# LucasAlegre/morl-baselines

Measured on NVIDIA B200. Metric: envelope_q_updates_per_sec, higher is better.
Workload: dtype f32

## Files before the change

### include/morl_b200.h

```cpp
#ifndef MORL_B200_H_
#define MORL_B200_H_

#include <stddef.h>
#include <stdint.h>

#ifdef __cplusplus
extern "C" {
#endif

#define MORL_B200_VERSION 100

#if defined(__GNUC__)
#define MORL_API __attribute__((visibility("default")))
#else
#define MORL_API
#endif

#define MORL_OK 0
#define MORL_ERR_NULL (-1)
#define MORL_ERR_SHAPE (-2)
#define MORL_ERR_ALIGN (-3)
#define MORL_ERR_UNSUPPORTED (-4)
#define MORL_ERR_NO_DEVICE (-5)

// ... 66 lines not shown
                                 void* stream);
MORL_API int morl_front_unpack_f64(const double* gathered, int world, int d, int cap, int n_extra, double* pts_out, double* meta_out, void* stream);

MORL_API int morl_hypervolume_f64(const double* pts, const uint8_t* keep, int n, int d, const double* ref, double* out, void* stream);

MORL_API int morl_polyak_f32(const float* const* params, float* const* targets, const int64_t* sizes, int n_tensors,
                    int64_t max_size, double tau, void* stream);


MORL_API int morl_sumtree_walk_f64(const double* tree, int n_levels, const double* u, int n, int scale_by_root, long long* out_index, void* stream);
MORL_API int morl_sumtree_batch_set_f64(double* tree, int n_levels, const long long* index, const double* priority, int n, int* err_flag,
                                        void* stream);
MORL_API int morl_sumtree_set_f64(double* tree, int n_levels, long long index, double priority, int use_min_priority, const double* min_priority,
                                  int* err_flag, void* stream);
MORL_API int morl_per_priority_f32(const float* raw, int n, float alpha, double* min_priority, double* prio64, float* prio32, void* stream);

#define MORL_FMT_BF16X3 0
#define MORL_FMT_F16X2 1
#define MORL_SPLIT_MAX_JOBS 16
typedef struct MorlSplitJob {
    const float* src;
    void* dst_planes;
    long long plane_stride;
    float* scale;
    int rows, cols, ld_src, transpose, rows_pad, ldp;
    int auto_scale, target_exp;
} MorlSplitJob;
MORL_API int morl_plane_overflow_count(int reset);
MORL_API int morl_amax_scale_f32(const float* src, long long n, int target_exp, float* scale_out, void* workspace, void* stream);
MORL_API int morl_split_planes_multi(int fmt, const MorlSplitJob* jobs, int n_jobs, void* stream);
// ... 72 lines not shown
```

### morl_baselines_b200/_lib.py

```python

from __future__ import annotations

import ctypes as C
import os

HERE = os.path.dirname(os.path.abspath(__file__))
LIB_PATH = os.path.join(HERE, "csrc", "libmorl_b200.so")

DOT_UNFUSED, DOT_FMA, DOT_PAIRFMA = 0, 1, 2
MAP_TILE, MAP_BLOCK = 0, 1
ROWS_REFERENCE, ROWS_BMAJOR = 0, 1
AC_ELEMENTWISE_MIN, AC_SCALAR_MIN, AC_ARGMIN_GATHER = 0, 1, 2
MAX_D = 8
FMT_BF16X3, FMT_F16X2 = 0, 1

_vp, _i, _f, _d, _i64, _sz = C.c_void_p, C.c_int, C.c_float, C.c_double, C.c_int64, C.c_size_t

SIGNATURES = {
    "morl_version": (_i, []),
    "morl_last_error": (C.c_char_p, []),
    "morl_device_sm_count": (_i, []),
    "morl_envelope_td_f32": (_i, [_vp, _vp, _vp, _vp, _vp, _f, _i, _i, _i, _i, _i, _i, _vp, _vp, _vp, _vp]),
    "morl_greedy_td_f32": (_i, [_vp, _vp, _vp, _i, _i, _vp, _vp, _i, _i, _f, _i, _i, _i, _i, _vp, _vp, _vp]),
    "morl_critic_min_td_f32": (_i, [_vp, _i, _vp, _i, _i, _vp, _vp, _i, _i, _f, _i, _i, _i, _i, _vp, _vp, _vp]),
    "morl_gpi_envelope_f32": (_i, [_vp, _i, _vp, _i, _i, _vp, _vp, _i, _i, _f, _i, _i, _i, _i, _i, _vp, _vp, _vp, _vp]),
    "morl_actor_critic_td_f32": (_i, [_vp, _i, _vp, _i, _i, _vp, _vp, _vp, _f, _f, _i, _i, _i, _vp, _vp]),
    "morl_td_workspace_bytes": (_sz, [_i]),
    "morl_td_mse_priority_f32": (_i, [_vp, _vp, _vp, _vp, _f, _vp, _i, _i, _i, _i, _i, _vp, _vp, _vp, _vp, _vp, _vp]),
    "morl_td_huber_priority_f32": (_i, [_vp, _i, _vp, _i, _vp, _vp, _vp, _i, _i, _f, _i, _i, _i, _i, _vp, _vp, _vp, _vp, _vp]),
    "morl_host_sumtree_walk": (_i, [_vp, _i, _vp, _i, _vp]),
    "morl_host_sumtree_batch_set": (_i, [_vp, _i, _vp, _vp, _i]),
    "morl_host_gather_rows": (_i, [_vp, C.c_longlong, _vp, _i, _vp]),
    "morl_host_gather_u8_to_i32": (_i, [_vp, C.c_longlong, _vp, _i, _vp]),
    "morl_sumtree_walk_f64": (_i, [_vp, _i, _vp, _i, _i, _vp, _vp]),
    "morl_sumtree_batch_set_f64": (_i, [_vp, _i, _vp, _vp, _i, _vp, _vp]),
    "morl_sumtree_set_f64": (_i, [_vp, _i, C.c_longlong, _d, _i, _vp, _vp, _vp]),
    "morl_per_priority_f32": (_i, [_vp, _i, _f, _vp, _vp, _vp, _vp]),
    "morl_replay_gather": (_i, [_vp, _vp, _vp, _vp, _vp, _vp, _i, _i, _i, _i, _i, _i64, _vp, _vp, _vp, _vp, _vp, _vp]),
    "morl_pareto_mask_f32": (_i, [_vp, _i, _i, _i, _vp, _vp]),
    "morl_pareto_mask_f64": (_i, [_vp, _i, _i, _i, _vp, _vp]),
    "morl_front_pack_f64": (_i, [_vp, _vp, _i, _i, _i, _vp, _i, _vp, _vp]),
    "morl_front_unpack_f64": (_i, [_vp, _i, _i, _i, _i, _vp, _vp, _vp]),
    "morl_hypervolume_f64": (_i, [_vp, _vp, _i, _i, _vp, _vp, _vp]),
    "morl_polyak_f32": (_i, [_vp, _vp, _vp, _i, _i64, _d, _vp]),
    "morl_plane_overflow_count": (_i, [_i]),
    "morl_amax_scale_f32": (_i, [_vp, C.c_longlong, _i, _vp, _vp, _vp]),
    "morl_split_planes_multi": (_i, [_i, _vp, _i, _vp]),
    "morl_split_planes": (_i, [_i, _vp, _i, _i, _i, _i, _vp, _i, _i, C.c_longlong, _vp, _vp]),
    "morl_gemm_planes_f32": (_i, [_i, _vp, C.c_longlong, _vp, _vp, C.c_longlong, _vp, _i, _i, _i, _i, _vp, _i, _vp, _i, _vp, _i, _vp, _i, C.c_longlong,
                                  _vp, _i, _i, _vp, _vp, _vp]),
    "morl_gemm_chain_supported": (_i, [_i, _i, _i]),
    "morl_gemm_chain_f32": (_i, [_i, _i, _i, _vp, C.c_longlong, _vp, _vp, C.c_longlong, _vp, _vp, _i, _vp, _vp, _i, _i, _i, _vp]),
# ... 69 lines not shown
```

### morl_baselines_b200/common/prioritized_buffer.py

```python

from __future__ import annotations

import numpy as np
import torch as th

from .. import _lib
from .buffer import ReplayBuffer, ReplayBufferSamplesNp


class SumTree:

    def __init__(self, max_size):
        self.n_levels = int(np.ceil(np.log2(max_size))) + 1
        self._alloc(np.zeros((1 << self.n_levels) - 1))

    def _alloc(self, flat):
        self._flat = np.ascontiguousarray(flat, dtype=np.float64)
        self.nodes = [self._flat[(1 << l) - 1 : (1 << (l + 1)) - 1] for l in range(self.n_levels)]
        self._lib = _lib.load()

    def __getstate__(self):
        return {"n_levels": self.n_levels, "flat": self._flat}

    def __setstate__(self, state):
# ... 154 lines not shown
            obs, act, rew, nobs, done = self.gather_device(idxes)
            return obs, act, rew, nobs, done, th.from_numpy(idxes)
        tup = ReplayBufferSamplesNp(self.obs[idxes], self.actions[idxes], self.rewards[idxes], self.next_obs[idxes], self.dones[idxes], idxes)
        if to_tensor:
            return tuple(map(lambda x: th.tensor(x).to(device), tup))
        return tup

    def sample_obs(self, batch_size, to_tensor=False, device=None):
        idxes = self.tree.sample(batch_size)
        return th.tensor(self.obs[idxes]).to(device) if to_tensor else self.obs[idxes]

    def update_priorities(self, idxes, priorities):
        self.min_priority = max(self.min_priority, priorities.max())
        self.tree.batch_set(np.asarray(idxes), priorities)

    def update_priorities_dev(self, idx_dev, raw_dev, alpha: float, prio64_dev, prio32_dev=None):
        if not self.tree_on_device:
            raise _lib.MorlB200Error("update_priorities_dev needs tree_on_device=True")
        lib = _lib.load()
        st = th.cuda.current_stream().cuda_stream
        _lib.check(lib.morl_per_priority_f32(raw_dev.data_ptr(), raw_dev.shape[0], float(alpha), self._min_p_dev.data_ptr(), prio64_dev.data_ptr(),
                                             None if prio32_dev is None else prio32_dev.data_ptr(), st), "morl_per_priority_f32")
        self.tree.batch_set_dev(idx_dev, prio64_dev)

    def get_all_data(self, max_samples=None, to_tensor=False, device=None):
        if max_samples is not None and max_samples < self.size:
            inds = np.random.choice(self.size, max_samples, replace=False)
        else:
            inds = np.arange(self.size)
        tup = (self.obs[inds], self.actions[inds], self.rewards[inds], self.next_obs[inds], self.dones[inds])
        if to_tensor:
            return tuple(map(lambda x: th.tensor(x).to(device), tup))
        return tup
```

### morl_baselines_b200/csrc/api.cu

```cuda
#include <stdlib.h>
#include <stdarg.h>
#include <string.h>

#include "common.cuh"

namespace morl {

static thread_local char g_err[512] = "";

void set_error(const char* fmt, ...) {
    va_list ap;
    va_start(ap, fmt);
    vsnprintf(g_err, sizeof(g_err), fmt, ap);
    va_end(ap);
}

int check_launch(const char* what) {
    cudaError_t e = cudaPeekAtLastError();
    if (e != cudaSuccess) {
        (void)cudaGetLastError();
        set_error("%s: %s", what, cudaGetErrorString(e));
        return static_cast<int>(e);
    }
    return MORL_OK;
}

bool pdl_enabled() {
    static const bool on = [] { const char* e = getenv("MORL_PDL"); return e && e[0] == '1'; }();
    return on;
}

}

extern "C" {

int morl_version(void) { return MORL_B200_VERSION; }

const char* morl_last_error(void) { return morl::g_err; }

int morl_device_sm_count(void) {
    int dev = 0;
    cudaError_t e = cudaGetDevice(&dev);
    if (e != cudaSuccess) {
        (void)cudaGetLastError();
        morl::set_error("morl_device_sm_count: no CUDA device (%s)", cudaGetErrorString(e));
        return MORL_ERR_NO_DEVICE;
// ... 13 lines not shown
```

### morl_baselines_b200/csrc/common.cuh

```cuda
#pragma once
#include <cuda_runtime.h>
#include <math.h>
#include <stdint.h>
#include <stdio.h>
#include <string.h>

#include "../../include/morl_b200.h"

namespace morl {

void set_error(const char* fmt, ...);
int check_launch(const char* what);

#define MORL_REQUIRE(cond, code, ...)    \
    do {                                 \
        if (!(cond)) {                   \
            ::morl::set_error(__VA_ARGS__); \
            return (code);               \
        }                                \
    } while (0)

static inline bool aligned16(const void* p) { return (reinterpret_cast<uintptr_t>(p) & 15u) == 0; }

__device__ __forceinline__ void pdl_enter() {
    asm volatile("griddepcontrol.launch_dependents;" ::: "memory");
    asm volatile("griddepcontrol.wait;" ::: "memory");
}

bool pdl_enabled();

template <typename... KArgs, typename... Args>
static inline void launch_k(void (*kernel)(KArgs...), dim3 grid, dim3 block, size_t smem, cudaStream_t stream, Args&&... args) {
    cudaLaunchConfig_t cfg;
    memset(&cfg, 0, sizeof(cfg));
    cfg.gridDim = grid;
    cfg.blockDim = block;
    cfg.dynamicSmemBytes = smem;
    cfg.stream = stream;
    cudaLaunchAttribute attr[1];
    attr[0].id = cudaLaunchAttributeProgrammaticStreamSerialization;
    attr[0].val.programmaticStreamSerializationAllowed = 1;
    cfg.attrs = attr;
    cfg.numAttrs = pdl_enabled() ? 1 : 0;
    cudaLaunchKernelEx(&cfg, kernel, static_cast<KArgs>(args)...);
// ... 79 lines not shown
```

### morl_baselines_b200/csrc/gemm_planes.cu

```cuda
#include <cuda.h>
#include <cuda_bf16.h>
#include <cuda_fp16.h>
#include <stdlib.h>
#include <string.h>

#include "common.cuh"
#include "gemm_tc.cuh"

namespace morl {

constexpr int kGemmBM = 128;
constexpr int kGemmThreads = 320;

__device__ unsigned int g_plane_overflow;


__device__ __forceinline__ void note_overflow(float amax) {
    if (amax > 65504.f) atomicAdd(&g_plane_overflow, 1u);
}

#define MORL_DISPATCH_FMT(F_, ...)                                                         \
    switch (F_) {                                                                          \
        case MORL_FMT_BF16X3: { constexpr int kFmt = MORL_FMT_BF16X3; __VA_ARGS__; } break; \
        case MORL_FMT_F16X2: { constexpr int kFmt = MORL_FMT_F16X2; __VA_ARGS__; } break;   \
// ... 1249 lines not shown
#pragma unroll
    for (int j = 0; j < 8; ++j) red[threadIdx.y][threadIdx.x][j] = acc[j];
    __syncthreads();
    if (threadIdx.y == 0 && h0 < H) {
#pragma unroll
        for (int j = 0; j < 8; ++j) {
            float t = 0.f;
#pragma unroll
            for (int y = 0; y < 8; ++y) t += red[y][threadIdx.x][j];
            dU[(size_t)b * H + h0 + j] = t * inv;
        }
    }
}

constexpr int kPgrMaxB = 8;
template <int FMT>
__global__ void __launch_bounds__(256, 2) pairs_grad_reduce_fused_kernel(const uint16_t* __restrict__ planes, long long plane_stride, int B, int W,
                                                                      int H, int b_per_chunk, float* __restrict__ dU, float* __restrict__ partV,
                                                                      const float* __restrict__ scale) {
    pdl_enter();
    using F = PlaneFmt<FMT>;
    extern __shared__ float red_dyn[];
    const int h0 = (blockIdx.y * 32 + threadIdx.x) * 8;
    const int b0 = blockIdx.x * b_per_chunk, b1 = min(B, b0 + b_per_chunk);
    const float inv = 1.0f / ld_scale(scale);
    float accV[8][8];
#pragma unroll
    for (int k = 0; k < 8; ++k)
#pragma unroll
        for (int c = 0; c < 8; ++c) accV[k][c] = 0.f;
    for (int b = b0; b < b1; ++b) {
        float accU[8];
#pragma unroll
        for (int c = 0; c < 8; ++c) accU[c] = 0.f;
#pragma unroll
        for (int kk = 0; kk < 8; kk += 4) {
            uint4 ld[4][F::P];
#pragma unroll
            for (int q = 0; q < 4; ++q) {
                const int j = threadIdx.y + 8 * (kk + q);
                const bool ok = h0 < H && j < W;
                const size_t o = ok ? ((size_t)b * W + j) * H + h0 : 0;
#pragma unroll
                for (int p = 0; p < F::P; ++p)
                    ld[q][p] = ok ? __ldg(reinterpret_cast<const uint4*>(planes + p * plane_stride + o)) : make_uint4(0u, 0u, 0u, 0u);
            }
#pragma unroll
            for (int q = 0; q < 4; ++q) {
                float v[8];
#pragma unroll
                for (int c = 0; c < 8; ++c) v[c] = 0.f;
#pragma unroll
                for (int p = 0; p < F::P; ++p) F::add8(v, ld[q][p]);
#pragma unroll
                for (int c = 0; c < 8; ++c) {
                    accU[c] += v[c];
                    accV[kk + q][c] += v[c];
                }
            }
        }
        float* r = red_dyn + (((size_t)(b - b0) * 8 + threadIdx.y) * 32 + threadIdx.x) * 9;
#pragma unroll
        for (int c = 0; c < 8; ++c) r[c] = accU[c];
    }
    __syncthreads();
    if (h0 < H) {
        for (int bl = threadIdx.y; bl < b1 - b0; bl += 8) {
#pragma unroll
            for (int c = 0; c < 8; ++c) {
                float t = 0.f;
#pragma unroll
                for (int y = 0; y < 8; ++y) t += red_dyn[(((size_t)bl * 8 + y) * 32 + threadIdx.x) * 9 + c];
                dU[(size_t)(b0 + bl) * H + h0 + c] = t * inv;
            }
        }
#pragma unroll
        for (int k = 0; k < 8; ++k) {
            const int j = threadIdx.y + 8 * k;
            if (j < W) {
                float* dst = partV + ((size_t)blockIdx.x * W + j) * H + h0;
                *reinterpret_cast<float4*>(dst) = make_float4(accV[k][0], accV[k][1], accV[k][2], accV[k][3]);
                *reinterpret_cast<float4*>(dst + 4) = make_float4(accV[k][4], accV[k][5], accV[k][6], accV[k][7]);
            }
        }
    }
}

__device__ __forceinline__ float scale_from_amax(float amax, int target_exp) {
    if (!(amax > 0.f) || !isfinite(amax)) return 1.0f;
    int e;
    (void)frexpf(amax, &e);
    int k = target_exp - e;
    k = k < -60 ? -60 : (k > 60 ? 60 : k);
    return ldexpf(1.0f, k);
}

__global__ void __launch_bounds__(256) amax_scale_kernel(const float* __restrict__ src, long long n, int target_exp, float* __restrict__ scale_out,
// ... 482 lines not shown
extern "C" int morl_pairs_grad_reduce_planes(int fmt, const void* planes, long long plane_stride, const float* scale, int B, int W, int H, float* dU,
                                             float* dV, void* workspace, void* stream) {
    using namespace morl;
    MORL_REQUIRE(fmt_ok(fmt), MORL_ERR_UNSUPPORTED, "morl_pairs_grad_reduce_planes: unknown plane format %d", fmt);
    MORL_REQUIRE(planes && dU && dV && workspace, MORL_ERR_NULL, "morl_pairs_grad_reduce_planes: NULL pointer argument");
    MORL_REQUIRE(B > 0 && W > 0 && H > 0 && H % 8 == 0 && plane_stride % 8 == 0, MORL_ERR_SHAPE, "morl_pairs_grad_reduce_planes: bad shape B=%d W=%d H=%d", B, W, H);
    cudaStream_t st = static_cast<cudaStream_t>(stream);
    const uint16_t* pl = static_cast<const uint16_t*>(planes);
    if (W <= 64) {
        int bpc = (B + 295) / 296;
        if (bpc > kPgrMaxB) bpc = kPgrMaxB;
        const int nchf = (B + bpc - 1) / bpc;
        if (nchf <= 296) {
            const int Nf = W * H;
            float* partf = static_cast<float*>(workspace);
            const size_t smemf = (size_t)kPgrMaxB * 8 * 32 * 9 * sizeof(float);
            MORL_DISPATCH_FMT(fmt, {
                static bool configured = false;
                if (!configured) {
                    cudaFuncSetAttribute(pairs_grad_reduce_fused_kernel<kFmt>, cudaFuncAttributeMaxDynamicSharedMemorySize, (int)smemf);
                    configured = true;
                }
                launch_k(pairs_grad_reduce_fused_kernel<kFmt>, dim3(dim3((unsigned)nchf, (unsigned)((H + 255) / 256))), dim3(dim3(32, 8)), smemf, st, pl, plane_stride, B, W,
                                                                                                                                     H, bpc, dU, partf, scale);
            });
            int rcf = check_launch("morl_pairs_grad_reduce_planes(fused)");
            if (rcf) return rcf;
            launch_k(reduce_partials_kernel, dim3((Nf + 31) / 32), dim3(dim3(32, 8)), 0, st, partf, nchf, 1, Nf, 1, Nf, 0, dV, Nf, 1 << 30, nullptr, nullptr, scale, nullptr);
            return check_launch("morl_pairs_grad_reduce_planes(reduce)");
        }
    }
    MORL_DISPATCH_FMT(fmt, (pairs_rowblock_sum_kernel<kFmt><<<dim3((unsigned)B, (unsigned)((H + 255) / 256)), dim3(32, 8), 0, st>>>(pl, plane_stride, W, H,
                                                                                                                                     dU, scale)));
    int rc = check_launch("morl_pairs_grad_reduce_planes(dU)");
    if (rc) return rc;
    const int N = W * H;
    const int chunks = 74;
    const int rpc = (B + chunks - 1) / chunks;
    const int nch = (B + rpc - 1) / rpc;
// ... 322 lines not shown
```

### morl_baselines_b200/csrc/optim.cu

```cuda
#include "common.cuh"

namespace morl {

__global__ void __launch_bounds__(256) polyak_kernel(const float* const* __restrict__ params, float* const* __restrict__ targets,
                                                     const int64_t* __restrict__ sizes, float tau, float one_minus_tau) {
    pdl_enter();
    const int t = blockIdx.y;
    const int64_t n = sizes[t];
    const float* __restrict__ p = params[t];
    float* __restrict__ q = targets[t];
    const int64_t stride = (int64_t)gridDim.x * blockDim.x;
    for (int64_t e = (int64_t)blockIdx.x * blockDim.x + threadIdx.x; e < n; e += stride) {
        if (tau == 1.0f)
            q[e] = p[e];
        else
            q[e] = __fmaf_rn(tau, p[e], __fmul_rn(q[e], one_minus_tau));
    }
}

}

extern "C" int morl_polyak_f32(const float* const* params, float* const* targets, const int64_t* sizes, int n_tensors, int64_t max_size,
                               double tau, void* stream) {
    using namespace morl;
// ... 22 lines not shown
    const float* __restrict__ g = grads[t];
    float acc = 0.f;
    for (int64_t e = (int64_t)blockIdx.x * blockDim.x + threadIdx.x; e < n; e += (int64_t)gridDim.x * blockDim.x) acc += g[e] * g[e];
#pragma unroll
    for (int off = 16; off > 0; off >>= 1) acc += __shfl_xor_sync(0xffffffffu, acc, off);
    if ((threadIdx.x & 31) == 0) red[threadIdx.x >> 5] = acc;
    __syncthreads();
    if (threadIdx.x == 0) {
        float s = 0.f;
        for (int w = 0; w < kOptBlock / 32; ++w) s += red[w];
        partials[(size_t)t * gridDim.x + blockIdx.x] = s;
        if (blockIdx.x == 0) *steps[t] += 1.0f;
    }
}

__global__ void __launch_bounds__(kOptBlock) adam_clip_kernel(float* const* __restrict__ params, const float* const* __restrict__ grads,
                                                              float* const* __restrict__ exp_avg, float* const* __restrict__ exp_avg_sq,
                                                              float* const* __restrict__ steps, const int64_t* __restrict__ sizes,
                                                              const float* __restrict__ partials, int n_partials, float max_norm, float lr,
                                                              float beta1, float beta2, float eps) {
    pdl_enter();
    __shared__ float s_coef;
    __shared__ double s_red[kOptBlock / 32];
    if (max_norm > 0.f) {
        double tot = 0.0;
        for (int i = threadIdx.x; i < n_partials; i += kOptBlock) tot += (double)partials[i];
#pragma unroll
        for (int off = 16; off > 0; off >>= 1) tot += __shfl_xor_sync(0xffffffffu, tot, off);
        if ((threadIdx.x & 31) == 0) s_red[threadIdx.x >> 5] = tot;
        __syncthreads();
        if (threadIdx.x == 0) {
            double t2 = 0.0;
            for (int w = 0; w < kOptBlock / 32; ++w) t2 += s_red[w];
            const float total_norm = (float)sqrt(t2);
            s_coef = fminf(max_norm / (total_norm + 1e-6f), 1.0f);
        }
    } else if (threadIdx.x == 0) {
        s_coef = 1.0f;
// ... 35 lines not shown
extern "C" int morl_adam_clip_f32(float* const* params, const float* const* grads, float* const* exp_avg, float* const* exp_avg_sq,
                                  float* const* steps, const int64_t* sizes, int n_tensors, int64_t max_size, float max_grad_norm, float lr,
                                  float beta1, float beta2, float eps, void* workspace, void* stream) {
    using namespace morl;
    MORL_REQUIRE(params && grads && exp_avg && exp_avg_sq && steps && sizes && workspace, MORL_ERR_NULL, "morl_adam_clip_f32: NULL pointer argument");
    MORL_REQUIRE(n_tensors > 0 && n_tensors <= 65535 && max_size > 0, MORL_ERR_SHAPE, "morl_adam_clip_f32: bad n_tensors=%d max_size=%lld", n_tensors,
                 (long long)max_size);
    cudaStream_t st = static_cast<cudaStream_t>(stream);
    long long bx = (max_size + kOptBlock - 1) / kOptBlock;
    if (bx > 64) bx = 64;
    const dim3 grid((unsigned)bx, (unsigned)n_tensors, 1);
    float* partials = static_cast<float*>(workspace);
    launch_k(grad_sqnorm_kernel, dim3(grid), dim3(kOptBlock), 0, st, grads, sizes, steps, partials);
    int rc = check_launch("morl_adam_clip_f32(norm)");
    if (rc) return rc;
    launch_k(adam_clip_kernel, dim3(grid), dim3(kOptBlock), 0, st, params, grads, exp_avg, exp_avg_sq, steps, sizes, partials, (int)(bx * n_tensors), max_grad_norm, lr, beta1,
                                                 beta2, eps);
    return check_launch("morl_adam_clip_f32");
}
```

### morl_baselines_b200/csrc/pair_layer1.cu

```cuda
#include "common.cuh"

namespace morl {

constexpr int kL1Rows = 8;

__global__ void __launch_bounds__(256) pair_layer1_uv_kernel(const float* __restrict__ feats, const float* __restrict__ wset, const float* __restrict__ W1,
                                                             const float* __restrict__ b1, int B, int W, int F, int D, int H, float* __restrict__ u,
                                                             float* __restrict__ v) {
    pdl_enter();
    extern __shared__ float xs[];
    const int K = F + D;
    const int r0 = blockIdx.x * kL1Rows;
    const int kmax = F > D ? F : D;
    for (int t = threadIdx.x; t < kL1Rows * kmax; t += blockDim.x) {
        const int rr = t / kmax, k = t - rr * kmax;
        const int r = r0 + rr;
        float x = 0.f;
        if (r < B) {
            if (k < F) x = __ldg(feats + (size_t)r * F + k);
        } else if (r < B + W) {
            if (k < D) x = __ldg(wset + (size_t)(r - B) * D + k);
        }
        xs[t] = x;
    }
// ... 27 lines not shown
#pragma unroll
        for (int rr = 0; rr < kL1Rows; ++rr) {
            const int r = r0 + rr;
            if (r < B)
                u[(size_t)r * H + h] = accu[rr];
            else if (r < B + W)
                v[(size_t)(r - B) * H + h] = accu[rr];
        }
    }
}

constexpr int kL1Splits = 16;
constexpr int kL1Chunk = 32;
constexpr int kL1ColsPerThread = 8;

__global__ void __launch_bounds__(256) pair_layer1_grad_kernel(const float* __restrict__ dU, const float* __restrict__ dV, const float* __restrict__ feats,
                                                               const float* __restrict__ wset, int B, int W, int F, int D, int H, float* __restrict__ dW1,
                                                               float* __restrict__ db1, float* __restrict__ partial, unsigned int* __restrict__ counters) {
    pdl_enter();
    __shared__ float gs[kL1Chunk][33];
    __shared__ float xs[kL1Chunk][8 * kL1ColsPerThread + 1];
    __shared__ unsigned int s_last;
    const int C = F + D + 1;
    const int h0 = blockIdx.x * 32, s = blockIdx.y;
    const int hl = threadIdx.x & 31, grp = threadIdx.x >> 5;
    const int bs = (B + kL1Splits - 1) / kL1Splits, js = (W + kL1Splits - 1) / kL1Splits;
    for (int cb = 0; cb < C; cb += 8 * kL1ColsPerThread) {
        const int ncol = min(8 * kL1ColsPerThread, C - cb);
        float acc[kL1ColsPerThread];
#pragma unroll
        for (int k = 0; k < kL1ColsPerThread; ++k) acc[k] = 0.f;
        for (int phase = 0; phase < 2; ++phase) {
            const int lo = phase == 0 ? s * bs : s * js, hi = phase == 0 ? min(B, lo + bs) : min(W, lo + js);
            const int c_lo = phase == 0 ? 0 : F, c_hi = phase == 0 ? F : C;
            if (cb >= c_hi || cb + ncol <= c_lo) continue;
            const float* g = phase == 0 ? dU : dV;
            for (int r0 = lo; r0 < hi; r0 += kL1Chunk) {
                const int nr = min(kL1Chunk, hi - r0);
                __syncthreads();
                for (int t = threadIdx.x; t < nr * 32; t += 256) {
                    const int rr = t >> 5, hh = t & 31;
                    gs[rr][hh] = (h0 + hh < H) ? __ldg(g + (size_t)(r0 + rr) * H + h0 + hh) : 0.f;
                }
                for (int t = threadIdx.x; t < nr * 64; t += 256) {
                    const int rr = t >> 6, cl = t & 63, c = cb + cl;
                    float x = 0.f;
                    if (cl >= ncol) {
                    } else if (phase == 0) {
                        if (c < F) x = __ldg(feats + (size_t)(r0 + rr) * F + c);
                    } else {
                        if (c >= F && c < F + D) x = __ldg(wset + (size_t)(r0 + rr) * D + (c - F));
                        else if (c == F + D) x = 1.0f;
                    }
                    xs[rr][cl] = x;
                }
                __syncthreads();
                for (int rr = 0; rr < nr; ++rr) {
                    const float gv = gs[rr][hl];
#pragma unroll
                    for (int k = 0; k < kL1ColsPerThread; ++k) acc[k] = __fmaf_rn(gv, xs[rr][grp + 8 * k], acc[k]);
                }
            }
        }
        if (h0 + hl < H) {
#pragma unroll
            for (int k = 0; k < kL1ColsPerThread; ++k) {
                const int c = cb + grp + 8 * k;
                if (grp + 8 * k < ncol) partial[((size_t)s * H + h0 + hl) * C + c] = acc[k];
            }
// ... 57 lines not shown

extern "C" size_t morl_pair_layer1_grad_workspace_bytes(int F, int D, int H) {
    using namespace morl;
    if (F <= 0 || D <= 0 || H <= 0) return 0;
    return ((size_t)kL1Splits * H * (F + D + 1) + (size_t)(H + 31) / 32 + 4) * sizeof(float);
}

extern "C" int morl_pair_layer1_grad_f32(const float* dU, const float* dV, const float* feats, const float* wset, int B, int W, int F, int D, int H,
                                         float* dW1, float* db1, void* workspace, void* stream) {
    using namespace morl;
    MORL_REQUIRE(dU && dV && feats && wset && dW1 && db1 && workspace, MORL_ERR_NULL, "morl_pair_layer1_grad_f32: NULL pointer argument");
    MORL_REQUIRE(B > 0 && W > 0 && F > 0 && D > 0 && H > 0, MORL_ERR_SHAPE, "morl_pair_layer1_grad_f32: bad shape B=%d W=%d F=%d D=%d H=%d", B, W, F, D, H);
    float* partial = static_cast<float*>(workspace);
    unsigned int* counters = reinterpret_cast<unsigned int*>(partial + (size_t)kL1Splits * H * (F + D + 1));
    dim3 grid((H + 31) / 32, kL1Splits);
    launch_k(pair_layer1_grad_kernel, dim3(grid), dim3(256), 0, static_cast<cudaStream_t>(stream), dU, dV, feats, wset, B, W, F, D, H, dW1, db1, partial, counters);
    return check_launch("morl_pair_layer1_grad_f32");
}
```

### morl_baselines_b200/csrc/sumtree.cu

```cuda
#include "common.cuh"

namespace morl {

__device__ __forceinline__ double* st_level(double* tree, int l) { return tree + (((size_t)1) << l) - 1; }
__device__ __forceinline__ const double* st_level(const double* tree, int l) { return tree + (((size_t)1) << l) - 1; }

__global__ void __launch_bounds__(256) sumtree_walk_kernel(const double* __restrict__ tree, int n_levels, const double* __restrict__ u, int n,
                                                           int scale_by_root, long long* __restrict__ out) {
    pdl_enter();
    const int i = blockIdx.x * blockDim.x + threadIdx.x;
    if (i >= n) return;
    double q = scale_by_root ? __dmul_rn(tree[0], u[i]) : u[i];
    long long node = 0;
    for (int l = 1; l < n_levels; ++l) {
        const double left = st_level(tree, l)[2 * node];
        const bool right = q > left;
        node = 2 * node + (right ? 1 : 0);
        q = __dsub_rn(q, __dmul_rn(left, right ? 1.0 : 0.0));
    }
    out[i] = node;
}

constexpr int kStMaxBatch = 2048;
constexpr int kStThreads = 1024;
// ... 63 lines not shown
    __syncthreads();
    const int m = m_s;
    const long long total = (long long)n_levels * m;
    for (long long w = threadIdx.x; w < total; w += blockDim.x) {
        const int l = (int)(w / m), i = (int)(w - (long long)l * m);
        const int shift = n_levels - 1 - l;
        const int node = leaf[i] >> shift;
        if (i > 0 && (leaf[i - 1] >> shift) == node) continue;
        double* p = st_level(tree, l) + node;
        double acc = *p;
        for (int j = i; j < m && (leaf[j] >> shift) == node; ++j) acc = __dadd_rn(acc, diff[j]);
        *p = acc;
    }
}

__global__ void __launch_bounds__(32) sumtree_set_kernel(double* __restrict__ tree, int n_levels, long long index, double priority, int use_min,
                                                         const double* __restrict__ min_priority, int* __restrict__ err) {
    const long long n_leaves = (long long)1 << (n_levels - 1);
    if (index < 0 || index >= n_leaves) {
        if (threadIdx.x == 0) *err = 1;
        return;
    }
    const double p = use_min ? *min_priority : priority;
    const double d = __dsub_rn(p, st_level(tree, n_levels - 1)[index]);
    __syncwarp();
    for (int l = threadIdx.x; l < n_levels; l += 32) {
        double* node = st_level(tree, l) + (index >> (n_levels - 1 - l));
        *node = __dadd_rn(*node, d);
    }
}
// ... 30 lines not shown
    using namespace morl;
    MORL_REQUIRE(tree && u && out_index, MORL_ERR_NULL, "morl_sumtree_walk_f64: NULL pointer argument");
    MORL_REQUIRE(n_levels >= 1 && n_levels <= 31 && n >= 0, MORL_ERR_SHAPE, "morl_sumtree_walk_f64: bad shape n_levels=%d n=%d", n_levels, n);
    if (n == 0) return MORL_OK;
    launch_k(sumtree_walk_kernel, dim3((n + 255) / 256), dim3(256), 0, static_cast<cudaStream_t>(stream), tree, n_levels, u, n, scale_by_root, out_index);
    return check_launch("morl_sumtree_walk_f64");
}

extern "C" int morl_sumtree_batch_set_f64(double* tree, int n_levels, const long long* index, const double* priority, int n, int* err_flag,
                                          void* stream) {
    using namespace morl;
    MORL_REQUIRE(tree && index && priority && err_flag, MORL_ERR_NULL, "morl_sumtree_batch_set_f64: NULL pointer argument");
    MORL_REQUIRE(n_levels >= 1 && n_levels <= 31 && n >= 0 && n <= kStMaxBatch, MORL_ERR_SHAPE,
                 "morl_sumtree_batch_set_f64: bad shape n_levels=%d n=%d (at most %d indices per call)", n_levels, n, kStMaxBatch);
    if (n == 0) return MORL_OK;
    launch_k(sumtree_batch_set_kernel, dim3(1), dim3(kStThreads), 0, static_cast<cudaStream_t>(stream), tree, n_levels, index, priority, n, err_flag);
    return check_launch("morl_sumtree_batch_set_f64");
}

extern "C" int morl_sumtree_set_f64(double* tree, int n_levels, long long index, double priority, int use_min_priority, const double* min_priority,
                                    int* err_flag, void* stream) {
    using namespace morl;
    MORL_REQUIRE(tree && err_flag && (min_priority || !use_min_priority), MORL_ERR_NULL, "morl_sumtree_set_f64: NULL pointer argument");
    MORL_REQUIRE(n_levels >= 1 && n_levels <= 31, MORL_ERR_SHAPE, "morl_sumtree_set_f64: bad n_levels=%d", n_levels);
    sumtree_set_kernel<<<1, 32, 0, static_cast<cudaStream_t>(stream)>>>(tree, n_levels, index, priority, use_min_priority, min_priority, err_flag);
    return check_launch("morl_sumtree_set_f64");
}

extern "C" int morl_per_priority_f32(const float* raw, int n, float alpha, double* min_priority, double* prio64, float* prio32, void* stream) {
    using namespace morl;
    MORL_REQUIRE(raw && min_priority && prio64, MORL_ERR_NULL, "morl_per_priority_f32: NULL pointer argument");
    MORL_REQUIRE(n > 0, MORL_ERR_SHAPE, "morl_per_priority_f32: bad n=%d", n);
    launch_k(per_priority_kernel, dim3(1), dim3(kStThreads), 0, static_cast<cudaStream_t>(stream), raw, n, alpha, min_priority, prio64, prio32);
    return check_launch("morl_per_priority_f32");
}
```

Measured before the change: 1642.

## Add fast-tail path: fused PER priority/sumtree update, faster tail kernels

Adds an env-gated fast path, on by default, that touches several separate tail kernels. It fuses the PER priority computation with a new sumtree batch-set kernel that sorts indices bitonically and updates each tree node once per run. It also launches Adam one tensor per grid row, skipping empty blocks, and batches global loads in the layer-1 grad kernel. Finally, it moves the wide accumulator of the pairs grad-reduce kernel into shared memory for two-plane formats. The aim is fewer launches and less serialized tree work, at the cost of more shared memory and complexity.

```diff
diff --git a/include/morl_b200.h b/include/morl_b200.h
--- a/include/morl_b200.h
+++ b/include/morl_b200.h
@@ -104,6 +104,8 @@
 MORL_API int morl_sumtree_set_f64(double* tree, int n_levels, long long index, double priority, int use_min_priority, const double* min_priority,
                                   int* err_flag, void* stream);
 MORL_API int morl_per_priority_f32(const float* raw, int n, float alpha, double* min_priority, double* prio64, float* prio32, void* stream);
+MORL_API int morl_per_priority_batch_set_f64(double* tree, int n_levels, const long long* index, const float* raw, int n, float alpha,
+                                             double* min_priority, double* prio64, float* prio32, int* err_flag, void* stream);
 
 #define MORL_FMT_BF16X3 0
 #define MORL_FMT_F16X2 1
diff --git a/morl_baselines_b200/_lib.py b/morl_baselines_b200/_lib.py
--- a/morl_baselines_b200/_lib.py
+++ b/morl_baselines_b200/_lib.py
@@ -6,6 +6,7 @@
 
 HERE = os.path.dirname(os.path.abspath(__file__))
 LIB_PATH = os.path.join(HERE, "csrc", "libmorl_b200.so")
+FAST_TAIL = os.environ.get("MORL_FAST_TAIL", "1") != "0"
 
 DOT_UNFUSED, DOT_FMA, DOT_PAIRFMA = 0, 1, 2
 MAP_TILE, MAP_BLOCK = 0, 1
@@ -36,6 +37,7 @@
     "morl_sumtree_batch_set_f64": (_i, [_vp, _i, _vp, _vp, _i, _vp, _vp]),
     "morl_sumtree_set_f64": (_i, [_vp, _i, C.c_longlong, _d, _i, _vp, _vp, _vp]),
     "morl_per_priority_f32": (_i, [_vp, _i, _f, _vp, _vp, _vp, _vp]),
+    "morl_per_priority_batch_set_f64": (_i, [_vp, _i, _vp, _vp, _i, _f, _vp, _vp, _vp, _vp, _vp]),
     "morl_replay_gather": (_i, [_vp, _vp, _vp, _vp, _vp, _vp, _i, _i, _i, _i, _i, _i64, _vp, _vp, _vp, _vp, _vp, _vp]),
     "morl_pareto_mask_f32": (_i, [_vp, _i, _i, _i, _vp, _vp]),
     "morl_pareto_mask_f64": (_i, [_vp, _i, _i, _i, _vp, _vp]),
diff --git a/morl_baselines_b200/common/prioritized_buffer.py b/morl_baselines_b200/common/prioritized_buffer.py
--- a/morl_baselines_b200/common/prioritized_buffer.py
+++ b/morl_baselines_b200/common/prioritized_buffer.py
@@ -192,11 +192,18 @@
         self.min_priority = max(self.min_priority, priorities.max())
         self.tree.batch_set(np.asarray(idxes), priorities)
 
-    def update_priorities_dev(self, idx_dev, raw_dev, alpha: float, prio64_dev, prio32_dev=None):
+    def update_priorities_dev(self, idx_dev, raw_dev, alpha: float, prio64_dev, prio32_dev=None, fused=None):
         if not self.tree_on_device:
             raise _lib.MorlB200Error("update_priorities_dev needs tree_on_device=True")
         lib = _lib.load()
         st = th.cuda.current_stream().cuda_stream
+        if (_lib.FAST_TAIL if fused is None else fused) and idx_dev.shape[0] <= DeviceSumTree.MAX_BATCH:
+            t = self.tree
+            _lib.check(lib.morl_per_priority_batch_set_f64(t.flat.data_ptr(), t.n_levels, idx_dev.data_ptr(), raw_dev.data_ptr(), raw_dev.shape[0],
+                                                           float(alpha), self._min_p_dev.data_ptr(), prio64_dev.data_ptr(),
+                                                           None if prio32_dev is None else prio32_dev.data_ptr(), t.err.data_ptr(), st),
+                       "morl_per_priority_batch_set_f64")
+            return
         _lib.check(lib.morl_per_priority_f32(raw_dev.data_ptr(), raw_dev.shape[0], float(alpha), self._min_p_dev.data_ptr(), prio64_dev.data_ptr(),
                                              None if prio32_dev is None else prio32_dev.data_ptr(), st), "morl_per_priority_f32")
         self.tree.batch_set_dev(idx_dev, prio64_dev)
diff --git a/morl_baselines_b200/csrc/api.cu b/morl_baselines_b200/csrc/api.cu
--- a/morl_baselines_b200/csrc/api.cu
+++ b/morl_baselines_b200/csrc/api.cu
@@ -30,6 +30,11 @@
     return on;
 }
 
+bool fast_tail_enabled() {
+    static const bool on = [] { const char* e = getenv("MORL_FAST_TAIL"); return !(e && e[0] == '0'); }();
+    return on;
+}
+
 }
 
 extern "C" {
diff --git a/morl_baselines_b200/csrc/common.cuh b/morl_baselines_b200/csrc/common.cuh
--- a/morl_baselines_b200/csrc/common.cuh
+++ b/morl_baselines_b200/csrc/common.cuh
@@ -28,6 +28,7 @@
 }
 
 bool pdl_enabled();
+bool fast_tail_enabled();
 
 template <typename... KArgs, typename... Args>
 static inline void launch_k(void (*kernel)(KArgs...), dim3 grid, dim3 block, size_t smem, cudaStream_t stream, Args&&... args) {
diff --git a/morl_baselines_b200/csrc/gemm_planes.cu b/morl_baselines_b200/csrc/gemm_planes.cu
--- a/morl_baselines_b200/csrc/gemm_planes.cu
+++ b/morl_baselines_b200/csrc/gemm_planes.cu
@@ -1287,30 +1287,38 @@
 }
 
 constexpr int kPgrMaxB = 8;
-template <int FMT>
+template <int FMT, bool kWide>
 __global__ void __launch_bounds__(256, 2) pairs_grad_reduce_fused_kernel(const uint16_t* __restrict__ planes, long long plane_stride, int B, int W,
                                                                       int H, int b_per_chunk, float* __restrict__ dU, float* __restrict__ partV,
                                                                       const float* __restrict__ scale) {
     pdl_enter();
     using F = PlaneFmt<FMT>;
     extern __shared__ float red_dyn[];
+    constexpr int kRows = (kWide && F::P == 2) ? 8 : 4;
     const int h0 = (blockIdx.y * 32 + threadIdx.x) * 8;
     const int b0 = blockIdx.x * b_per_chunk, b1 = min(B, b0 + b_per_chunk);
     const float inv = 1.0f / ld_scale(scale);
-    float accV[8][8];
-#pragma unroll
-    for (int k = 0; k < 8; ++k)
-#pragma unroll
-        for (int c = 0; c < 8; ++c) accV[k][c] = 0.f;
+    const int tid = threadIdx.y * 32 + threadIdx.x;
+    float* accS = red_dyn + (size_t)b_per_chunk * 8 * 32 * 9 + tid;
+    float accV[kWide ? 1 : 8][8];
+    if constexpr (kWide) {
+#pragma unroll
+        for (int k = 0; k < 64; ++k) accS[k * 256] = 0.f;
+    } else {
+#pragma unroll
+        for (int k = 0; k < 8; ++k)
+#pragma unroll
+            for (int c = 0; c < 8; ++c) accV[k][c] = 0.f;
+    }
     for (int b = b0; b < b1; ++b) {
         float accU[8];
 #pragma unroll
         for (int c = 0; c < 8; ++c) accU[c] = 0.f;
 #pragma unroll
-        for (int kk = 0; kk < 8; kk += 4) {
-            uint4 ld[4][F::P];
-#pragma unroll
-            for (int q = 0; q < 4; ++q) {
+        for (int kk = 0; kk < 8; kk += kRows) {
+            uint4 ld[kRows][F::P];
+#pragma unroll
+            for (int q = 0; q < kRows; ++q) {
                 const int j = threadIdx.y + 8 * (kk + q);
                 const bool ok = h0 < H && j < W;
                 const size_t o = ok ? ((size_t)b * W + j) * H + h0 : 0;
@@ -1319,7 +1327,7 @@
                     ld[q][p] = ok ? __ldg(reinterpret_cast<const uint4*>(planes + p * plane_stride + o)) : make_uint4(0u, 0u, 0u, 0u);
             }
 #pragma unroll
-            for (int q = 0; q < 4; ++q) {
+            for (int q = 0; q < kRows; ++q) {
                 float v[8];
 #pragma unroll
                 for (int c = 0; c < 8; ++c) v[c] = 0.f;
@@ -1328,7 +1336,10 @@
 #pragma unroll
                 for (int c = 0; c < 8; ++c) {
                     accU[c] += v[c];
-                    accV[kk + q][c] += v[c];
+                    if constexpr (kWide)
+                        accS[((kk + q) * 8 + c) * 256] += v[c];
+                    else
+                        accV[kk + q][c] += v[c];
                 }
             }
         }
@@ -1352,8 +1363,14 @@
             const int j = threadIdx.y + 8 * k;
             if (j < W) {
                 float* dst = partV + ((size_t)blockIdx.x * W + j) * H + h0;
-                *reinterpret_cast<float4*>(dst) = make_float4(accV[k][0], accV[k][1], accV[k][2], accV[k][3]);
-                *reinterpret_cast<float4*>(dst + 4) = make_float4(accV[k][4], accV[k][5], accV[k][6], accV[k][7]);
+                if constexpr (kWide) {
+                    const float* a = accS + k * 8 * 256;
+                    *reinterpret_cast<float4*>(dst) = make_float4(a[0], a[256], a[512], a[768]);
+                    *reinterpret_cast<float4*>(dst + 4) = make_float4(a[1024], a[1280], a[1536], a[1792]);
+                } else {
+                    *reinterpret_cast<float4*>(dst) = make_float4(accV[k][0], accV[k][1], accV[k][2], accV[k][3]);
+                    *reinterpret_cast<float4*>(dst + 4) = make_float4(accV[k][4], accV[k][5], accV[k][6], accV[k][7]);
+                }
             }
         }
     }
@@ -1866,15 +1883,18 @@
         if (nchf <= 296) {
             const int Nf = W * H;
             float* partf = static_cast<float*>(workspace);
-            const size_t smemf = (size_t)kPgrMaxB * 8 * 32 * 9 * sizeof(float);
+            const bool wide = fast_tail_enabled();
+            const size_t smemf = wide ? (size_t)bpc * 8 * 32 * 9 * sizeof(float) + 64 * 256 * sizeof(float) : (size_t)kPgrMaxB * 8 * 32 * 9 * sizeof(float);
+            const size_t smem_max = (size_t)kPgrMaxB * 8 * 32 * 9 * sizeof(float) + 64 * 256 * sizeof(float);
             MORL_DISPATCH_FMT(fmt, {
                 static bool configured = false;
                 if (!configured) {
-                    cudaFuncSetAttribute(pairs_grad_reduce_fused_kernel<kFmt>, cudaFuncAttributeMaxDynamicSharedMemorySize, (int)smemf);
+                    cudaFuncSetAttribute(pairs_grad_reduce_fused_kernel<kFmt, false>, cudaFuncAttributeMaxDynamicSharedMemorySize, (int)smem_max);
+                    cudaFuncSetAttribute(pairs_grad_reduce_fused_kernel<kFmt, true>, cudaFuncAttributeMaxDynamicSharedMemorySize, (int)smem_max);
                     configured = true;
                 }
-                launch_k(pairs_grad_reduce_fused_kernel<kFmt>, dim3(dim3((unsigned)nchf, (unsigned)((H + 255) / 256))), dim3(dim3(32, 8)), smemf, st, pl, plane_stride, B, W,
-                                                                                                                                     H, bpc, dU, partf, scale);
+                launch_k(wide ? pairs_grad_reduce_fused_kernel<kFmt, true> : pairs_grad_reduce_fused_kernel<kFmt, false>,
+                         dim3(dim3((unsigned)nchf, (unsigned)((H + 255) / 256))), dim3(dim3(32, 8)), smemf, st, pl, plane_stride, B, W, H, bpc, dU, partf, scale);
             });
             int rcf = check_launch("morl_pairs_grad_reduce_planes(fused)");
             if (rcf) return rcf;
diff --git a/morl_baselines_b200/csrc/optim.cu b/morl_baselines_b200/csrc/optim.cu
--- a/morl_baselines_b200/csrc/optim.cu
+++ b/morl_baselines_b200/csrc/optim.cu
@@ -60,6 +60,7 @@
     }
 }
 
+template <bool kOneEach>
 __global__ void __launch_bounds__(kOptBlock) adam_clip_kernel(float* const* __restrict__ params, const float* const* __restrict__ grads,
                                                               float* const* __restrict__ exp_avg, float* const* __restrict__ exp_avg_sq,
                                                               float* const* __restrict__ steps, const int64_t* __restrict__ sizes,
@@ -68,6 +69,7 @@
     pdl_enter();
     __shared__ float s_coef;
     __shared__ double s_red[kOptBlock / 32];
+    if (kOneEach && (int64_t)blockIdx.x * blockDim.x >= sizes[blockIdx.y]) return;
     if (max_norm > 0.f) {
         double tot = 0.0;
         for (int i = threadIdx.x; i < n_partials; i += kOptBlock) tot += (double)partials[i];
@@ -133,7 +135,14 @@
     launch_k(grad_sqnorm_kernel, dim3(grid), dim3(kOptBlock), 0, st, grads, sizes, steps, partials);
     int rc = check_launch("morl_adam_clip_f32(norm)");
     if (rc) return rc;
-    launch_k(adam_clip_kernel, dim3(grid), dim3(kOptBlock), 0, st, params, grads, exp_avg, exp_avg_sq, steps, sizes, partials, (int)(bx * n_tensors), max_grad_norm, lr, beta1,
+    if (fast_tail_enabled()) {
+        long long bx1 = (max_size + kOptBlock - 1) / kOptBlock;
+        if (bx1 > 65535) bx1 = 65535;
+        launch_k(adam_clip_kernel<true>, dim3((unsigned)bx1, (unsigned)n_tensors, 1), dim3(kOptBlock), 0, st, params, grads, exp_avg, exp_avg_sq, steps, sizes,
+                 (const float*)partials, (int)(bx * n_tensors), max_grad_norm, lr, beta1, beta2, eps);
+        return check_launch("morl_adam_clip_f32");
+    }
+    launch_k(adam_clip_kernel<false>, dim3(grid), dim3(kOptBlock), 0, st, params, grads, exp_avg, exp_avg_sq, steps, sizes, partials, (int)(bx * n_tensors), max_grad_norm, lr, beta1,
                                                  beta2, eps);
     return check_launch("morl_adam_clip_f32");
 }
diff --git a/morl_baselines_b200/csrc/pair_layer1.cu b/morl_baselines_b200/csrc/pair_layer1.cu
--- a/morl_baselines_b200/csrc/pair_layer1.cu
+++ b/morl_baselines_b200/csrc/pair_layer1.cu
@@ -65,6 +65,7 @@
 constexpr int kL1Chunk = 32;
 constexpr int kL1ColsPerThread = 8;
 
+template <bool kBatched>
 __global__ void __launch_bounds__(256) pair_layer1_grad_kernel(const float* __restrict__ dU, const float* __restrict__ dV, const float* __restrict__ feats,
                                                                const float* __restrict__ wset, int B, int W, int F, int D, int H, float* __restrict__ dW1,
                                                                float* __restrict__ db1, float* __restrict__ partial, unsigned int* __restrict__ counters) {
@@ -89,6 +90,37 @@
             for (int r0 = lo; r0 < hi; r0 += kL1Chunk) {
                 const int nr = min(kL1Chunk, hi - r0);
                 __syncthreads();
+                if constexpr (kBatched) {
+                    float gr[kL1Chunk * 32 / 256], xr[kL1Chunk * 64 / 256];
+#pragma unroll
+                    for (int q = 0; q < kL1Chunk * 32 / 256; ++q) {
+                        const int t = threadIdx.x + 256 * q, rr = t >> 5, hh = t & 31;
+                        gr[q] = (rr < nr && h0 + hh < H) ? __ldg(g + (size_t)(r0 + rr) * H + h0 + hh) : 0.f;
+                    }
+#pragma unroll
+                    for (int q = 0; q < kL1Chunk * 64 / 256; ++q) {
+                        const int t = threadIdx.x + 256 * q, rr = t >> 6, cl = t & 63, c = cb + cl;
+                        float x = 0.f;
+                        if (rr >= nr || cl >= ncol) {
+                        } else if (phase == 0) {
+                            if (c < F) x = __ldg(feats + (size_t)(r0 + rr) * F + c);
+                        } else {
+                            if (c >= F && c < F + D) x = __ldg(wset + (size_t)(r0 + rr) * D + (c - F));
+                            else if (c == F + D) x = 1.0f;
+                        }
+                        xr[q] = x;
+                    }
+#pragma unroll
+                    for (int q = 0; q < kL1Chunk * 32 / 256; ++q) {
+                        const int t = threadIdx.x + 256 * q;
+                        if ((t >> 5) < nr) gs[t >> 5][t & 31] = gr[q];
+                    }
+#pragma unroll
+                    for (int q = 0; q < kL1Chunk * 64 / 256; ++q) {
+                        const int t = threadIdx.x + 256 * q;
+                        if ((t >> 6) < nr) xs[t >> 6][t & 63] = xr[q];
+                    }
+                } else {
                 for (int t = threadIdx.x; t < nr * 32; t += 256) {
                     const int rr = t >> 5, hh = t & 31;
                     gs[rr][hh] = (h0 + hh < H) ? __ldg(g + (size_t)(r0 + rr) * H + h0 + hh) : 0.f;
@@ -104,6 +136,7 @@
                         else if (c == F + D) x = 1.0f;
                     }
                     xs[rr][cl] = x;
+                }
                 }
                 __syncthreads();
                 for (int rr = 0; rr < nr; ++rr) {
@@ -191,6 +224,6 @@
     float* partial = static_cast<float*>(workspace);
     unsigned int* counters = reinterpret_cast<unsigned int*>(partial + (size_t)kL1Splits * H * (F + D + 1));
     dim3 grid((H + 31) / 32, kL1Splits);
-    launch_k(pair_layer1_grad_kernel, dim3(grid), dim3(256), 0, static_cast<cudaStream_t>(stream), dU, dV, feats, wset, B, W, F, D, H, dW1, db1, partial, counters);
+    launch_k(fast_tail_enabled() ? pair_layer1_grad_kernel<true> : pair_layer1_grad_kernel<false>, dim3(grid), dim3(256), 0, static_cast<cudaStream_t>(stream), dU, dV, feats, wset, B, W, F, D, H, dW1, db1, partial, counters);
     return check_launch("morl_pair_layer1_grad_f32");
 }
diff --git a/morl_baselines_b200/csrc/sumtree.cu b/morl_baselines_b200/csrc/sumtree.cu
--- a/morl_baselines_b200/csrc/sumtree.cu
+++ b/morl_baselines_b200/csrc/sumtree.cu
@@ -101,6 +101,181 @@
     }
 }
 
+constexpr int kStTopLevels = 10;
+
+__device__ __forceinline__ int st_lower_bound(const int* a, int n, int v) {
+    int lo = 0;
+    while (n > 0) {
+        const int h = n >> 1;
+        if (a[lo + h] < v) {
+            lo += h + 1;
+            n -= h + 1;
+        } else {
+            n = h;
+        }
+    }
+    return lo;
+}
+
+__device__ __forceinline__ double st_add_run(double acc, const double* diff, int lo, int hi) {
+    int j = lo;
+    for (; j + 16 <= hi; j += 16) {
+        double d[16];
+#pragma unroll
+        for (int k = 0; k < 16; ++k) d[k] = diff[j + k];
+#pragma unroll
+        for (int k = 0; k < 16; ++k) acc = __dadd_rn(acc, d[k]);
+    }
+    for (; j < hi; ++j) acc = __dadd_rn(acc, diff[j]);
+    return acc;
+}
+
+template <bool kPrio>
+__global__ void __launch_bounds__(kStThreads) sumtree_batch_set_fast_kernel(double* __restrict__ tree, int n_levels, const long long* __restrict__ idx,
+                                                                             const double* prio, int n, int* __restrict__ err, const float* __restrict__ raw,
+                                                                             float alpha, double* __restrict__ min_priority, double* p64, float* __restrict__ p32) {
+    pdl_enter();
+    __shared__ unsigned long long keyA[kStMaxBatch];
+    __shared__ __align__(16) unsigned char regionB[kStMaxBatch * 12];
+    __shared__ int wcnt[64];
+    __shared__ float red[kStThreads / 32];
+    unsigned long long* keyB = reinterpret_cast<unsigned long long*>(regionB);
+    double* diff = reinterpret_cast<double*>(regionB);
+    int* leaf = reinterpret_cast<int*>(regionB + kStMaxBatch * sizeof(double));
+    const int tid = threadIdx.x, lane = tid & 31, wid = tid >> 5;
+    if constexpr (kPrio) {
+        const double mp64 = *min_priority;
+        const float mp = (float)mp64;
+        float mx = 0.f;
+        for (int i = tid; i < n; i += kStThreads) {
+            const float x = __fadd_rn(raw[i], mp);
+            const float p = (float)pow((double)x, (double)alpha);
+            if (p32) p32[i] = p;
+            p64[i] = (double)p;
+            mx = fmaxf(mx, p);
+        }
+#pragma unroll
+        for (int off = 16; off > 0; off >>= 1) mx = fmaxf(mx, __shfl_xor_sync(0xffffffffu, mx, off));
+        if (lane == 0) red[wid] = mx;
+        __syncthreads();
+        if (tid < 32) {
+            mx = red[tid];
+#pragma unroll
+            for (int off = 16; off > 0; off >>= 1) mx = fmaxf(mx, __shfl_xor_sync(0xffffffffu, mx, off));
+            if (tid == 0 && (double)mx > mp64) *min_priority = (double)mx;
+        }
+        prio = p64;
+    }
+    const long long n_leaves = (long long)1 << (n_levels - 1);
+    int np2 = 1;
+    while (np2 < n) np2 <<= 1;
+    unsigned long long k2[2];
+#pragma unroll
+    for (int q = 0; q < 2; ++q) {
+        const int i = tid + q * kStThreads;
+        unsigned long long k = ~0ULL;
+        if (i < n) {
+            const long long v = idx[i];
+            if (v < 0 || v >= n_leaves)
+                *err = 1;
+            else
+                k = ((unsigned long long)v << 13) | (unsigned long long)i;
+        }
+        k2[q] = k;
+    }
+    const int nq = np2 > kStThreads ? 2 : 1;
+    int par = 0;
+    for (int size = 2; size <= np2; size <<= 1) {
+        for (int stride = size >> 1; stride > 0; stride >>= 1) {
+            if (stride == kStThreads) {
+                const unsigned long long a = k2[0], b = k2[1];
+                k2[0] = a < b ? a : b;
+                k2[1] = a < b ? b : a;
+            } else if (stride >= 32) {
+                unsigned long long* buf = par ? keyB : keyA;
+                par ^= 1;
+                for (int q = 0; q < nq; ++q) buf[tid + q * kStThreads] = k2[q];
+                __syncthreads();
+                for (int q = 0; q < nq; ++q) {
+                    const int i = tid + q * kStThreads;
+                    const unsigned long long a = k2[q], b = buf[i ^ stride];
+                    const bool want_min = ((i & stride) == 0) == ((i & size) == 0);
+                    k2[q] = want_min ? (a < b ? a : b) : (a < b ? b : a);
+                }
+            } else {
+                for (int q = 0; q < nq; ++q) {
+                    const int i = tid + q * kStThreads;
+                    const unsigned long long a = k2[q], b = __shfl_xor_sync(0xffffffffu, a, stride);
+                    const bool want_min = ((i & stride) == 0) == ((i & size) == 0);
+                    k2[q] = want_min ? (a < b ? a : b) : (a < b ? b : a);
+                }
+            }
+        }
+    }
+    __syncthreads();
+    for (int q = 0; q < 2; ++q) keyA[tid + q * kStThreads] = k2[q];
+    __syncthreads();
+    bool head[2];
+#pragma unroll
+    for (int q = 0; q < 2; ++q) {
+        const int i = tid + q * kStThreads;
+        head[q] = i < n && k2[q] != ~0ULL && (i == 0 || (k2[q] >> 13) != (keyA[i - 1] >> 13));
+        const unsigned bal = __ballot_sync(0xffffffffu, head[q]);
+        if (lane == 0) wcnt[q * 32 + wid] = __popc(bal);
+    }
+    __syncthreads();
+    if (wid == 0) {
+        const int c0 = wcnt[2 * lane], c1 = wcnt[2 * lane + 1];
+        int incl = c0 + c1;
+#pragma unroll
+        for (int off = 1; off < 32; off <<= 1) {
+            const int v = __shfl_up_sync(0xffffffffu, incl, off);
+            if (lane >= off) incl += v;
+        }
+        const int excl = incl - c0 - c1;
+        wcnt[2 * lane] = excl;
+        wcnt[2 * lane + 1] = excl + c0;
+        if (lane == 31) red[0] = __int_as_float(incl);
+    }
+    __syncthreads();
+    const int m = __float_as_int(red[0]);
+    const double* leaves = st_level(tree, n_levels - 1);
+#pragma unroll
+    for (int q = 0; q < 2; ++q) {
+        const unsigned bal = __ballot_sync(0xffffffffu, head[q]);
+        if (head[q]) {
+            const int pos = wcnt[q * 32 + wid] + __popc(bal & ((1u << lane) - 1u));
+            const int lf = (int)(k2[q] >> 13);
+            leaf[pos] = lf;
+            diff[pos] = __dsub_rn(__ldcg(prio + (k2[q] & 0x1FFFULL)), leaves[lf]);
+        }
+    }
+    __syncthreads();
+    const int top = n_levels < kStTopLevels ? n_levels : kStTopLevels;
+    if (tid < (1 << top) - 1) {
+        const int l = 31 - __clz(tid + 1);
+        const int node = tid + 1 - (1 << l);
+        const int shift = n_levels - 1 - l;
+        const int lo = st_lower_bound(leaf, m, node << shift);
+        const int hi = lo + st_lower_bound(leaf + lo, m - lo, (node + 1) << shift);
+        if (lo < hi) {
+            double* p = st_level(tree, l) + node;
+            *p = st_add_run(*p, diff, lo, hi);
+        }
+    }
+    const int total = (n_levels - top) * m;
+    for (int w = tid; w < total; w += kStThreads) {
+        const int l = top + w / m, i = w % m;
+        const int shift = n_levels - 1 - l;
+        const int node = leaf[i] >> shift;
+        if (i > 0 && (leaf[i - 1] >> shift) == node) continue;
+        int hi = i + 1;
+        while (hi < m && (leaf[hi] >> shift) == node) ++hi;
+        double* p = st_level(tree, l) + node;
+        *p = st_add_run(*p, diff, i, hi);
+    }
+}
+
 __global__ void __launch_bounds__(32) sumtree_set_kernel(double* __restrict__ tree, int n_levels, long long index, double priority, int use_min,
                                                          const double* __restrict__ min_priority, int* __restrict__ err) {
     const long long n_leaves = (long long)1 << (n_levels - 1);
@@ -161,7 +336,11 @@
     MORL_REQUIRE(n_levels >= 1 && n_levels <= 31 && n >= 0 && n <= kStMaxBatch, MORL_ERR_SHAPE,
                  "morl_sumtree_batch_set_f64: bad shape n_levels=%d n=%d (at most %d indices per call)", n_levels, n, kStMaxBatch);
     if (n == 0) return MORL_OK;
-    launch_k(sumtree_batch_set_kernel, dim3(1), dim3(kStThreads), 0, static_cast<cudaStream_t>(stream), tree, n_levels, index, priority, n, err_flag);
+    if (fast_tail_enabled())
+        launch_k(sumtree_batch_set_fast_kernel<false>, dim3(1), dim3(kStThreads), 0, static_cast<cudaStream_t>(stream), tree, n_levels, index, priority, n,
+                 err_flag, (const float*)nullptr, 0.f, (double*)nullptr, (double*)nullptr, (float*)nullptr);
+    else
+        launch_k(sumtree_batch_set_kernel, dim3(1), dim3(kStThreads), 0, static_cast<cudaStream_t>(stream), tree, n_levels, index, priority, n, err_flag);
     return check_launch("morl_sumtree_batch_set_f64");
 }
 
@@ -181,3 +360,14 @@
     launch_k(per_priority_kernel, dim3(1), dim3(kStThreads), 0, static_cast<cudaStream_t>(stream), raw, n, alpha, min_priority, prio64, prio32);
     return check_launch("morl_per_priority_f32");
 }
+
+extern "C" int morl_per_priority_batch_set_f64(double* tree, int n_levels, const long long* index, const float* raw, int n, float alpha,
+                                               double* min_priority, double* prio64, float* prio32, int* err_flag, void* stream) {
+    using namespace morl;
+    MORL_REQUIRE(tree && index && raw && min_priority && prio64 && err_flag, MORL_ERR_NULL, "morl_per_priority_batch_set_f64: NULL pointer argument");
+    MORL_REQUIRE(n_levels >= 1 && n_levels <= 31 && n > 0 && n <= kStMaxBatch, MORL_ERR_SHAPE,
+                 "morl_per_priority_batch_set_f64: bad shape n_levels=%d n=%d (at most %d indices per call)", n_levels, n, kStMaxBatch);
+    launch_k(sumtree_batch_set_fast_kernel<true>, dim3(1), dim3(kStThreads), 0, static_cast<cudaStream_t>(stream), tree, n_levels, index,
+             (const double*)prio64, n, err_flag, raw, alpha, min_priority, prio64, prio32);
+    return check_launch("morl_per_priority_batch_set_f64");
+}
```

After: 1668, median of 6. 1.02x the previous value.
